# hasindu2008/cornetto

Hardware: AMD Instinct MI355X
Metric: Gbases/s scanned (telowin+sdust+boringbits) (higher is better)
Workload: dtype u8/u16 integer

## Files before the change

### cornetto_amd/__init__.py

```python
import ctypes as C
import os

import numpy as np

__all__ = ["lib", "Accel", "AccelError", "HIT_DT", "WIN_DT", "IVL_DT", "TELROW_DT", "khash_str_order", "panel_boring", "REG_DT", "REGREC_DT", "build",
           "LIB_PATH", "CLI_PATH"]

HERE = os.path.dirname(os.path.abspath(__file__))
DEV_LIB_PATH = os.path.join(HERE, "libcornetto_hip_dev.so")
LIB_PATH = os.environ.get("CORNETTO_LIB") or os.path.join(HERE, "libcornetto_hip.so")
CLI_PATH = os.path.join(HERE, "cornetto")

HIT_DT = np.dtype([("ctg", "<i4"), ("strand", "<i4"), ("start", "<i4"), ("end", "<i4")])
WIN_DT = np.dtype([("ctg", "<i4"), ("start", "<i4"), ("end", "<i4"), ("car", "<i4")])
IVL_DT = np.dtype([("ctg", "<i4"), ("start", "<i4"), ("finish", "<i4")])
TELROW_DT = np.dtype([("ctg", "<i4"), ("start", "<i4"), ("end", "<i4"), ("matched", "<i4")])
FQREC_DT = np.dtype([("head", "<i8"), ("seq", "<i8"), ("qual", "<i8"), ("len", "<i4"), ("name_len", "<i4"),
                     ("comment_len", "<i4"), ("keep", "<i4")])
EMITREC_DT = np.dtype([("ctg", "<i4"), ("rc", "<i4"), ("head", "<i8"), ("head_len", "<i8")])
FAREC_DT = np.dtype([("head", "<i8"), ("len", "<i8"), ("name_len", "<i4"), ("pad", "<i4")])
REG_DT = np.dtype([("st", "<i4"), ("end", "<i4"), ("depth", "<i4"), ("mq_depth", "<i4")])
REGREC_DT = np.dtype([("ctg", "<i4"), ("st", "<i4"), ("end", "<i4"), ("depth", "<i4"), ("mq_depth", "<i4")])
REGPK_DT = np.dtype([("st", "<i4"), ("depth", "<u2"), ("mq_depth", "<u2")])

# ... 343 lines not shown
    def telo_scan(self, asm, motif, thr_adj, want_hits=True):
        ph, nh, pw, nw = C.c_void_p(), C.c_int64(), C.c_void_p(), C.c_int64()
        self._chk(self.L.cornetto_telo_scan(self.h, asm.ptr, motif, thr_adj,
                                            C.byref(ph) if want_hits else None, C.byref(nh) if want_hits else None,
                                            C.byref(pw), C.byref(nw)))
        hits = _take(self.L, ph, nh.value, HIT_DT) if want_hits else None
        return hits, _take(self.L, pw, nw.value, WIN_DT)

    def sdust(self, asm, T=20, W=64):
        p, n = C.c_void_p(), C.c_int64()
        self._chk(self.L.cornetto_sdust_asm(self.h, asm.ptr, T, W, C.byref(p), C.byref(n)))
        return _take(self.L, p, n.value, IVL_DT)

    def sdust_begin(self, asm, T=20, W=64):
        self._chk(self.L.cornetto_sdust_asm_begin(self.h, asm.ptr, T, W))

    def sdust_end(self, asm, T=20, W=64):
        p, n = C.c_void_p(), C.c_int64()
        self._chk(self.L.cornetto_sdust_asm_end(self.h, asm.ptr, T, W, C.byref(p), C.byref(n)))
        return _take(self.L, p, n.value, IVL_DT)

    def sdust_stats(self, asm, T=20, W=64):
        self.L.cornetto_accel_sdust_stats(self.h, 1, None, 0)
        try:
            self.sdust(asm, T, W)
        finally:
            out = np.zeros(256, dtype=np.uint64)
            n = self.L.cornetto_accel_sdust_stats(self.h, 0, out.ctypes.data, 256)
        s = [int(x) for x in out[:n]]
        waves = s[254]
        if n > 207 and s[206]:
            return {"kernel": "sd_sift", "chunks": s[255], "tiles_of_64_bases": s[206], "positions_ct_above_T10": s[203], "after_L1": s[204], "after_L2": s[205],
                    "resolve_steps": s[200], "resolve_window_reads": s[201], "dp_tiles": s[208], "passes_with_candidates": s[202], "base_by_base_steps_of_chunks_with_other_bytes": s[207],
                    "window_reads_behind_a_gap_of": {"2": s[209], "3-4": s[210], "5-8": s[211]} if n > 211 else None}
        if not waves or not s[2]:
            return None
        hist = []
        for b in range(32):
            w = s[16 + 4 * b]
            if w:
                hist.append({"ms": [b * 0.5, b * 0.5 + 0.5], "waves": w, "jobs": s[18 + 4 * b], "find_perfect": s[19 + 4 * b], "find_perfect_with_candidates": s[17 + 4 * b]})
        return {"waves": waves, "chunks": s[255], "chunks_sampled_low_complexity": s[7], "wave_steps": s[2], "find_perfect_calls": s[3],
                "find_perfect_with_candidates": s[10], "plain_groups": s[4], "wave_ms_avg": round(s[5] / waves / 1e5, 3), "wave_ms_max": round(s[6] / 1e5, 3),
                "queue_fetch_rounds_per_wave": round(s[11] / waves, 1), "wave_time_histogram": hist}

    def cov_select_merged(self, cov, lo, hi, low_mq, edge_len, min_ctg_len, boring, merge_dist=1000, min_len=30000):
        p, n = C.c_void_p(), C.c_int64()
        self._chk(self.L.cornetto_cov_select_merged(self.h, cov.ptr, lo, hi, low_mq, edge_len, min_ctg_len, 1 if boring else 0, merge_dist, min_len,
                                                    C.byref(p), C.byref(n)))
        return _take(self.L, p, n.value, IVL_DT)

    def ivl_merge(self, ivls, dist):
        ivls = np.ascontiguousarray(ivls, dtype=IVL_DT)
        p, n = C.c_void_p(), C.c_int64()
        self._chk(self.L.cornetto_ivl_merge(self.h, ivls.ctypes.data, len(ivls), dist, C.byref(p), C.byref(n)))
        return _take(self.L, p, n.value, IVL_DT)

    def telobreaks(self, ctg_len, sd, tel):
        ctg_len = np.ascontiguousarray(ctg_len, dtype=np.int32)
        sd = np.ascontiguousarray(sd, dtype=IVL_DT)
        tel = np.ascontiguousarray(tel, dtype=TELROW_DT)
        p, n = C.c_void_p(), C.c_int64()
        self._chk(self.L.cornetto_telobreaks(self.h, ctg_len.ctypes.data, len(ctg_len), sd.ctypes.data, len(sd), tel.ctypes.data, len(tel),
                                             C.byref(p), C.byref(n)))
        return _take(self.L, p, n.value, IVL_DT)

    def cov_upload(self, depths, mqs):
# ... 164 lines not shown
```

### cornetto_amd/csrc/sdust.hip

```cpp
#include <algorithm>
#include <type_traits>
#include <ctime>
#include <sched.h>

#include "common.hpp"
#include "scan.hpp"
#include "tiles.hpp"
#include "ivlmerge.hpp"

namespace {

__device__ __forceinline__ int nt4_code(uint32_t c);
struct SdArgs;
struct SdChunk;
template <bool LEAN = false>
__device__ int sd_find_start(const SdArgs &A, const SdChunk ch, const uint8_t *seq);

struct SdChunk {
    int32_t ctg, start, end;
};
struct SdChunkFill {
    SdChunk *out;
    const int32_t *len;
    int32_t chunk;
// ... 1574 lines not shown
            uint32_t *d_slots = (uint32_t *)cn_ws(h, WS_SD_OFF, (size_t)(std::max<int64_t>(sd_waves, 1) + SD_WPB) * 64 * 64 * sizeof(uint32_t));
            if (!d_slots) return cn_fail(h, CORNETTO_E_NOMEM, "sdust: workspace allocation failed");
            stamp("row + slot workspaces");
            const bool use_w64 = w64_path;
            SdArgs A{a->d_bases, a->d_off, a->d_len, d_chunks, (int32_t)nc, T, W, d_out, d_cnt, (uint32_t)cap,
                     want_stats ? d_tot + 2 : nullptr, reinterpret_cast<uint32_t *>(d_tot + 1), d_slots, nullptr,
                     reinterpret_cast<uint32_t *>(d_tot + 8), nullptr, 0, CN_DEV_INT("CORNETTO_SDUST_RUNON", 1), (int32_t)chunk, a->d_wtab, a->d_wtab_base, reinterpret_cast<uint32_t *>(d_tot + 1) + 1};
            unsigned nb = (unsigned)((nc + 63) / 64);
            bool sift_walk_pending = false;
            bool dense_pending = false;
            struct DenseJoin {
                cornetto_accel_t *h;
                bool *pending;
                ~DenseJoin() { if (*pending && h->stream2) (void)hipStreamSynchronize(h->stream2); }
            } dense_join{h, &dense_pending};
            if (use_w64 && sift_on) {
                CN_HIP(h, hipMemsetAsync(d_cnt, 0, nc * 4, h->stream));
                const uint32_t reg_cap = (uint32_t)(chunk + 128);
                const uint32_t lds_wave = sift_lds_bytes(reg_cap);
                int lmin = 1;
                while (5 * (lmin + 1) <= T && lmin < 16) ++lmin;
                const bool walk_known = a->d_sd_walk && a->sd_walk_key == key;
                const size_t walk_words = 2 + 4 * nc + ((nc + 4095) / 4096 + 2);
                if (!walk_known) {
                    if (a->d_sd_walk) { (void)hipFree(a->d_sd_walk); a->d_sd_walk = nullptr; }
                    a->sd_walk_key = -1;
                    if (cn_obj_malloc(h, (void **)&a->d_sd_walk, walk_words * 4) != hipSuccess) return cn_fail(h, CORNETTO_E_NOMEM, "sdust: device allocation failed");
                    CN_HIP(h, hipMemsetAsync(a->d_sd_walk, 0, (2 + 2 * nc) * 4, h->stream));
                }
                uint32_t *d_wflag = a->d_sd_walk + 2 + nc, *d_wrank = d_wflag + nc, *d_worder = d_wrank + nc, *d_wpart = d_worder + nc;
                SiftArgs S{a->d_bases, a->d_off, a->d_len, d_chunks, (int32_t)nc, T, W, lds_wave, reg_cap,
                           walk_known ? d_worder : nullptr, walk_known ? nullptr : a->d_sd_walk, walk_known ? nullptr : d_wflag,
                           reinterpret_cast<uint32_t *>(d_tot + 256), T / 10 + 1, lmin, CN_DEV_INT("CORNETTO_SIFT_ABL", 0),
                           std::min(65, std::max(1, CN_DEV_INT("CORNETTO_SIFT_DP", 24))), std::min(65, std::max(1, CN_DEV_INT("CORNETTO_SIFT_L2SKIP", 48)))};
                sift_walk_pending = !walk_known;
                SdArgs R = A;
                R.stats = want_stats ? d_tot + 200 : nullptr;
                const bool cap_default = reg_cap == SIFT_CAP_DEFAULT && !CN_DEV_INT("CORNETTO_SIFT_GENERIC", 0) && !CN_DEV_INT("CORNETTO_SIFT_ABL", 0);
                if (h->sift_per_cu == 0 || h->sift_per_cu_default != (cap_default ? 1 : 0)) {
                    int per_cu = 0;
                    const hipError_t oe = cap_default ? hipOccupancyMaxActiveBlocksPerMultiprocessor(&per_cu, sd_sift<false, SIFT_CAP_DEFAULT>, 64 * SIFT_WPB, lds_wave * SIFT_WPB)
                                                      : hipOccupancyMaxActiveBlocksPerMultiprocessor(&per_cu, sd_sift<false>, 64 * SIFT_WPB, lds_wave * SIFT_WPB);
                    if (oe != hipSuccess || per_cu < 1) per_cu = 8;
                    h->sift_per_cu = per_cu;
                    h->sift_per_cu_default = cap_default ? 1 : 0;
                }
                const int per_cu_all = std::max(1, std::min<int>(h->sift_per_cu, (int)(163840 / ((lds_wave * SIFT_WPB + 1279) / 1280 * 1280))));
                const bool free_now = __atomic_load_n(&h->boost, __ATOMIC_ACQUIRE) != 0;
                const size_t cus_n = (size_t)std::max(h->sd_cus, 1);
                const size_t slots_all = (size_t)per_cu_all * cus_n;
                const size_t slots = free_now ? slots_all : std::max<size_t>(cus_n, slots_all * (size_t)h->share / 100);
                const size_t all_blocks = (nc + SIFT_WPB - 1) / SIFT_WPB;
                const unsigned nbk = (unsigned)std::min<size_t>(all_blocks, (size_t)CN_DEV_INT("CORNETTO_SIFT_BLOCKS", (int)slots));
                const unsigned extra = (unsigned)std::min<size_t>(all_blocks > nbk ? all_blocks - nbk : 0, slots_all > slots ? slots_all - slots : 0);
                const bool may_help = phase == 0 && extra > 0 && !want_stats && h->share < CN_DEV_INT("CORNETTO_SDUST_HELP_BELOW", 70);
                if (may_help) {
                    if (!h->stream2) {
                        int pr_least = 0, pr_greatest = 0;
                        (void)hipDeviceGetStreamPriorityRange(&pr_least, &pr_greatest);
                        CN_HIP(h, hipStreamCreateWithPriority(&h->stream2, hipStreamNonBlocking, pr_greatest));
                        CN_HIP(h, hipEventCreateWithFlags(&h->ev2, hipEventDisableTiming));
                        CN_HIP(h, hipEventCreateWithFlags(&h->ev1, hipEventDisableTiming));
                    }
                    if (!h->ev3) CN_HIP(h, hipEventCreateWithFlags(&h->ev3, hipEventDisableTiming));
                    CN_HIP(h, hipEventRecord(h->ev1, h->stream));
                }
                stamp("set up");
                if (want_stats) CN_LAUNCH(h, "sdust_kernel", sd_sift<true><<<dim3(nbk), dim3(64 * SIFT_WPB), lds_wave * SIFT_WPB, h->stream>>>(S, R));
                else if (cap_default) CN_LAUNCH(h, "sdust_kernel", sd_sift<false, SIFT_CAP_DEFAULT><<<dim3(nbk), dim3(64 * SIFT_WPB), lds_wave * SIFT_WPB, h->stream>>>(S, R));
                else CN_LAUNCH(h, "sdust_kernel", sd_sift<false><<<dim3(nbk), dim3(64 * SIFT_WPB), lds_wave * SIFT_WPB, h->stream>>>(S, R));
                __atomic_fetch_add(&h->launch_seq, 1ull, __ATOMIC_RELEASE);
                if (may_help) {
                    CN_HIP(h, hipEventRecord(h->ev3, h->stream));
                    bool helped = false;
                    while (hipEventQuery(h->ev3) == hipErrorNotReady) {
                        if (!helped && __atomic_load_n(&h->boost, __ATOMIC_ACQUIRE) != 0) {
                            CN_HIP(h, hipStreamWaitEvent(h->stream2, h->ev1, 0));
                            if (cap_default) sd_sift<false, SIFT_CAP_DEFAULT><<<dim3(extra), dim3(64 * SIFT_WPB), lds_wave * SIFT_WPB, h->stream2>>>(S, R);
                            else sd_sift<false><<<dim3(extra), dim3(64 * SIFT_WPB), lds_wave * SIFT_WPB, h->stream2>>>(S, R);
                            dense_pending = true;
                            CN_HIP(h, hipGetLastError());
                            CN_HIP(h, hipEventRecord(h->ev2, h->stream2));
                            helped = true;
                        }
                        sched_yield();
                    }
                    if (helped) CN_HIP(h, hipStreamWaitEvent(h->stream, h->ev2, 0));
// ... 138 lines not shown
                        cornetto_free(of);
                        return cn_fail(h, CORNETTO_E_HIP, "sdust: stitch / copy back failed");
                    }
                    if (phase == 1) {
                        h->sd_pend.state = 1; h->sd_pend.a = a; h->sd_pend.T = T; h->sd_pend.W = W; h->sd_pend.of = of;
                        h->sd_pend.m_cap = m_cap; h->sd_pend.n_cap = n_cap; h->sd_pend.cap = cap; h->sd_pend.key = key; h->sd_pend.walk_pending = sift_walk_pending;
                        return CORNETTO_OK;
                    }
                    const int fin = sd_one_go_finish(h, a, of, p_tot, cap, n_cap, m_cap, key, sift_walk_pending, ivls, n_ivls);
                    if (fin <= 0) {
                        if (fin == 0) stamp("results on the host (one go)");
                        return fin;
                    }
                } else if (of) {
                    cornetto_free(of);
                }
            }
            stamp("main kernel queued");
            CN_HIP(h, hipMemcpyAsync(p_tot, d_tot, want_stats ? 2048 : 128, hipMemcpyDeviceToHost, h->stream));
            CN_HIP(h, hipStreamSynchronize(h->stream));
            stamp("main kernel done");
            if (want_stats) {
                memcpy(h->sd_last, p_tot, 2048);
                if (a->sd_flagged >= 0) h->sd_last[7] = (unsigned long long)a->sd_flagged;
                h->sd_last[254] = nb;
                h->sd_last[255] = nc;
            }
            if (env_stats)
                for (int b = 0; b < 32; ++b)
                    if (p_tot[16 + 4 * b])
                        fprintf(stderr, "[sdust stats]   waves that ran %4.1f-%4.1f ms: %6llu, job fetches %llu, find_perfect calls %llu (%llu with candidates)\n", b * 0.5, b * 0.5 + 0.5,
                                p_tot[16 + 4 * b], p_tot[18 + 4 * b], p_tot[19 + 4 * b], p_tot[17 + 4 * b]);
            if (env_stats && sift_on)
                fprintf(stderr, "[sdust stats] sift: tiles %llu, positions with ct > T/10 %llu, after L1 %llu, after L2 %llu; resolve: steps %llu, window reads %llu (behind a gap of 2 / 3-4 / 5-8: %llu / %llu / %llu), dp tiles %llu; passes with candidates %llu; base-by-base steps of chunks with other bytes %llu\n",
                        p_tot[206], p_tot[203], p_tot[204], p_tot[205], p_tot[200], p_tot[201], p_tot[209], p_tot[210], p_tot[211], p_tot[208], p_tot[202], p_tot[207]);
            if (env_stats)
                fprintf(stderr, "[sdust stats] flagged low-complexity %llu; chunks %zu waves %u wave-steps %llu find_perfect calls %llu (%llu with candidates) plain groups %llu; wave time avg %.1f us max %.1f us; queue: %.1f fetch rounds and %.1f us per wave\n", p_tot[7], nc, nb,
                        p_tot[2], p_tot[3], p_tot[10], p_tot[4], nb ? (double)p_tot[5] / nb / 100.0 : 0.0, (double)p_tot[6] / 100.0, nb ? (double)p_tot[11] / nb : 0.0, nb ? (double)p_tot[12] / nb / 100.0 : 0.0);
            const uint32_t ovf = (uint32_t)(p_tot[1] & 0xFFFFFFFFull);
            const bool need_wtab = (p_tot[1] >> 32) != 0;
            if (need_wtab) {
                if (a->d_wtab) return cn_fail(h, CORNETTO_E_HIP, "sdust: word-count table requested twice");
                std::vector<int64_t> base(a->n + 1, 0);
                for (int32_t c = 0; c < a->n; ++c) base[c + 1] = base[c] + a->len[c] / SD_WBLK + 2;
                a->n_wblocks = base[a->n];
                const size_t npart = ((size_t)a->n_wblocks + 4095) / 4096 + 1;
                uint32_t *d_wcnt = nullptr;
                if (hipMalloc((void **)&a->d_wtab, ((size_t)a->n_wblocks + 1) * 4) != hipSuccess ||
                    hipMalloc((void **)&a->d_wtab_base, ((size_t)a->n + 1) * 8) != hipSuccess ||
                    hipMalloc((void **)&d_wcnt, ((size_t)a->n_wblocks + npart + 1) * 4) != hipSuccess)
                    return cn_fail(h, CORNETTO_E_NOMEM, "sdust: word-count table allocation failed");
                CN_HIP(h, hipMemcpyAsync(a->d_wtab_base, base.data(), ((size_t)a->n + 1) * 8, hipMemcpyHostToDevice, h->stream));
                const unsigned nbw = (unsigned)((a->n_wblocks + 255) / 256);
                CN_LAUNCH(h, "sd_wordcount", sd_wordcount<<<dim3(nbw), dim3(256), 0, h->stream>>>(a->d_bases, a->d_off, a->d_len, a->d_wtab_base, a->n,
                                                                                         a->n_wblocks, d_wcnt));
                int rc = cnscan::exclusive_u32(h, "sd_wordscan", d_wcnt, a->n_wblocks, 1, a->d_wtab, d_wcnt + a->n_wblocks, nullptr);
                hipError_t e = hipStreamSynchronize(h->stream);
                (void)hipFree(d_wcnt);
                if (rc != CORNETTO_OK) return rc;
                if (e != hipSuccess) return cn_fail(h, CORNETTO_E_HIP, "sdust: word-count table build failed");
                continue;
            }
            if (sift_walk_pending && !need_wtab) a->sd_walk_key = key;
            if (ovf <= cap) {
                tot = p_tot[0];
                break;
            }
            if (attempt >= 2) return cn_fail(h, CORNETTO_E_HIP, "sdust: a chunk produced %u intervals after resizing to %zu", ovf, cap);
// ... 168 lines not shown
```

### cornetto_amd/csrc/sdust_sift.hpp

```cpp
#pragma once

struct SiftArgs {
    const uint8_t *bases;
    const int64_t *ctg_off;
    const int32_t *ctg_len;
    const SdChunk *chunks;
    int32_t n_chunks;
    int32_t T, W;
    uint32_t lds_per_wave;
    uint32_t reg_cap;
    const uint32_t *order;
    uint32_t *walk_out;
    uint32_t *iswalk_out;
    uint32_t *counter;
    int32_t thr, lmin;
    int32_t abl;
    int32_t dp_min;
    int32_t l2_skip;
};

#ifndef SIFT_WPB
#define SIFT_WPB 1
#endif
constexpr int SIFT_NCTR = 64;
constexpr int SIFT_PAD = 16;
#ifndef SIFT_K
#define SIFT_K 16
#endif
constexpr int SIFT_LS = SIFT_K - 1;
constexpr int SIFT_FIXED = 1024 + 512;
__host__ __device__ constexpr uint32_t sift_lds_bytes(uint32_t cap) { return (SIFT_FIXED + cap / 4 + 2 * (SIFT_PAD + cap) + 16 + 15) / 16 * 16; }


__device__ __forceinline__ uint32_t sd_codes4(uint32_t word)
{
    const uint32_t y = word & 0xDFDFDFDFu, idx = y & 0x07070707u;
    const uint32_t code = __builtin_amdgcn_perm(0x02000003u, 0x01000000u, idx);
    const uint32_t d = y ^ __builtin_amdgcn_perm(0x47FFFF54u, 0x43FF41FFu, idx);
    const uint32_t nz = ((d & 0x7F7F7F7Fu) + 0x7F7F7F7Fu) | d;
    return code | ((nz >> 5) & 0x04040404u);
}
__device__ __forceinline__ uint32_t sd_words4(uint32_t cn, uint32_t pcn)
{
    const uint32_t y1 = __builtin_amdgcn_alignbyte(cn, pcn, 3);
    const uint32_t y2 = __builtin_amdgcn_alignbyte(cn, pcn, 2);
    const uint32_t t = (cn & 0x03030303u) | ((y1 & 0x03030303u) << 2) | ((y2 & 0x03030303u) << 4);
    return t | (((cn | y1 | y2) & 0x04040404u) << 4);
}

__device__ __forceinline__ int sd_mbcnt64(unsigned long long m)
{
    return (int)__builtin_amdgcn_mbcnt_hi((uint32_t)(m >> 32), __builtin_amdgcn_mbcnt_lo((uint32_t)m, 0u));
}
__device__ __forceinline__ int sd_dpp_shr1(int old, int src, bool zero_fill)
{
    return zero_fill ? __builtin_amdgcn_update_dpp(0, src, 0x138, 0xF, 0xF, true) : __builtin_amdgcn_update_dpp(old, src, 0x138, 0xF, 0xF, false);
}
// ... 56 lines not shown
    uint8_t *const wc = L + SIFT_FIXED + cap / 4 + 2 * SIFT_PAD;
    const int T = A.T, W = A.W, CAPW = W - 2;

    const int lo = lane - (CAPW - 1);
    const unsigned long long below = lane ? ~0ull >> (64 - lane) : 0ull;
    const unsigned long long mc = lo > 0 ? below & (~0ull << lo) : below;
    const unsigned long long mp = lo < 0 ? ~0ull << (64 + lo) : 0ull;
    const uint32_t m_a = (uint32_t)mc, m_d = (uint32_t)(mp >> 32), m_m = lane < 32 ? (uint32_t)mp : (uint32_t)(mc >> 32);
    const uint32_t mybit = 1u << (lane & 31);
    uint32_t *const mine0 = tab + (lane < 32 ? 0 : 192), *const mine1 = tab + (lane < 32 ? 64 : 128);
    uint32_t *const tab_mine = mine0;
    const uint32_t *const mid1 = tab + (lane < 32 ? 0 : 128);
    const int thr = A.thr, lmin = A.lmin;
    const int LS = CAPW - 1 < SIFT_LS ? CAPW - 1 : SIFT_LS;
    const bool long_ok = CAPW - 1 > LS;
    unsigned long long st_steps = 0, st_jumps = 0, st_cand = 0, st_trig = 0, st_l1 = 0, st_l2 = 0, st_walk = 0, st_tiles = 0, st_dp = 0, st_g2 = 0, st_g4 = 0, st_g8 = 0;

    struct Meta {
        SdChunk ch;
        int len;
        const uint8_t *seq;
    };
    struct Data {
        uint4 q[2];
        uint32_t pw[2];
    };
    auto meta = [&](int kk) {
        Meta m;
        m.ch = A.chunks[kk];
        m.len = A.ctg_len[m.ch.ctg];
        m.seq = A.bases + A.ctg_off[m.ch.ctg];
        return m;
    };
    auto fetch = [&](const Meta &m) {
        Data d;
        const int rb = m.ch.start - (m.ch.start > 0 ? 128 : 0), rlen = m.ch.end - rb;
#pragma unroll
        for (int it = 0; it < 2; ++it) {
            const int b16 = lane * 16 + it * 1024;
            d.q[it] = make_uint4(0, 0, 0, 0);
            if (b16 < rlen) d.q[it] = *reinterpret_cast<const uint4 *>(m.seq + rb + b16);
        }
        uint32_t first = 0;
        if (rb > 0) first = *reinterpret_cast<const uint32_t *>(m.seq + rb - 4);
        d.pw[0] = (uint32_t)__builtin_amdgcn_update_dpp((int)first, (int)d.q[0].w, 0x138, 0xF, 0xF, false);
        d.pw[1] = (uint32_t)__builtin_amdgcn_update_dpp(rdlane((int)d.q[0].w, 63), (int)d.q[1].w, 0x138, 0xF, 0xF, false);
        return d;
    };

  auto process = [&](const int k, const Meta &M, const Data &D) {
    const SdChunk ch = M.ch;
    const int len = M.len;
    const uint8_t *seq = M.seq;
    const int halo = ch.start > 0 ? 128 : 0;
    const int rb = ch.start - halo;
    const int rlen = ch.end - rb;
    const int ntile = (rlen + 63) >> 6;
    const bool islast = ch.end == len;
    const int rec_from = ch.start;

    tab[lane] = 0;
    tab[64 + lane] = 0;
    tab[128 + lane] = 0;
    tab[192 + lane] = 0;
    for (int i = lane; i < (int)(cap >> 4); i += 64) sb[i] = 0;
    if (lane < SIFT_PAD) reinterpret_cast<uint16_t *>(wc)[lane - SIFT_PAD] = halo ? 0xFF40 : 0x0040;
    bool bad = false;
    bool general = rb <= 0 || rb + ((rlen + 15) & ~15) > len || (abl & 32);
    if (abl & 128) general = false;
    if (!general && !(abl & 128)) {
        uint32_t acc = 0u;
        int lane_s = lane * 16;
        for (int b16 = lane * 16, it = 0; it < STAGE_ROUNDS && b16 < rlen; b16 += 1024, ++it) {
            uint4 q;
            uint32_t pw;
            if (STAGE_ROUNDS <= 2 || it < 2) {
                q = D.q[it];
                pw = D.pw[it];
            } else {
                asm volatile("" : "+v"(lane_s));
                const uint8_t *const g = seq + rb + lane_s + it * 1024;
                q = *reinterpret_cast<const uint4 *>(g);
                pw = *reinterpret_cast<const uint32_t *>(g - 4);
            }
            const uint32_t ipw = pw & 0x07070707u;
            uint32_t pcn = __builtin_amdgcn_perm(0x02000003u, 0x01000000u, ipw);
            acc |= (pw & 0xDFDFDFDFu) ^ __builtin_amdgcn_perm(0x47FFFF54u, 0x43FF41FFu, ipw);
            const uint32_t in[4] = {q.x, q.y, q.z, q.w};
            uint32_t wo[8];
#pragma unroll
            for (int d = 0; d < 4; ++d) {
                const uint32_t idx = in[d] & 0x07070707u;
                const uint32_t cn = __builtin_amdgcn_perm(0x02000003u, 0x01000000u, idx);
                acc |= (in[d] & 0xDFDFDFDFu) ^ __builtin_amdgcn_perm(0x47FFFF54u, 0x43FF41FFu, idx);
                const uint32_t y1 = __builtin_amdgcn_alignbyte(cn, pcn, 3), y2 = __builtin_amdgcn_alignbyte(cn, pcn, 2);
                const uint32_t w4 = cn | y1 << 2 | y2 << 4;
                wo[2 * d] = __builtin_amdgcn_perm(0u, w4, 0x0C010C00u);
                wo[2 * d + 1] = __builtin_amdgcn_perm(0u, w4, 0x0C030C02u);
                pcn = cn;
            }
            uint4 *dst = reinterpret_cast<uint4 *>(wc + 2 * b16);
            dst[0] = make_uint4(wo[0], wo[1], wo[2], wo[3]);
            dst[1] = make_uint4(wo[4], wo[5], wo[6], wo[7]);
        }
        general = sd_any(acc != 0u);
    }
    if (general)
    for (int b16 = lane * 16, it = 0; it < STAGE_ROUNDS && b16 < rlen; b16 += 1024, ++it) {
        const int p0 = rb + b16;
        uint4 q;
        uint32_t pw;
        if (STAGE_ROUNDS <= 2 || it < 2) {
            q = D.q[it];
            pw = D.pw[it];
        } else {
            q = *reinterpret_cast<const uint4 *>(seq + p0);
            pw = *reinterpret_cast<const uint32_t *>(seq + p0 - 4);
        }
        uint32_t pcn = 0x04040404u;
        if (p0 > 0) pcn = sd_codes4(pw);
        const uint32_t in[4] = {q.x, q.y, q.z, q.w};
        uint32_t wo[8];
#pragma unroll
        for (int d = 0; d < 4; ++d) {
            uint32_t cn = sd_codes4(in[d]);
            if (p0 + 4 * d + 4 > len) {
                const int rem = len - (p0 + 4 * d);
                const uint32_t beyond = rem <= 0 ? 0xFFFFFFFFu : 0xFFFFFFFFu << (8 * rem);
                bad = bad || (cn & 0x04040404u & ~beyond) != 0u;
                cn |= 0x04040404u & beyond;
            } else {
                bad = bad || (cn & 0x04040404u) != 0u;
            }
            const uint32_t w4 = sd_words4(cn, pcn);
            wo[2 * d] = __builtin_amdgcn_perm(0u, w4, 0x0C010C00u);
            wo[2 * d + 1] = __builtin_amdgcn_perm(0u, w4, 0x0C030C02u);
            pcn = cn;
        }
        uint4 *dst = reinterpret_cast<uint4 *>(wc + 2 * b16);
        dst[0] = make_uint4(wo[0], wo[1], wo[2], wo[3]);
        dst[1] = make_uint4(wo[4], wo[5], wo[6], wo[7]);
    }
    const bool unclean = sd_any(bad);
    SD_LDS_ORDER();

    int w = 0, r = 0, slot = 0;
    int sv0 = 0;
    bool have_last = false;
    uint32_t last_s = 0, last_f = 0, n_out = 0;
    uint2 *const out = O.out + (size_t)k * O.cap;
    auto emit = [&](int ps, int pf, int tm) {
        if (tm < rec_from) return;
        if (have_last && ps <= (int)last_f) {
            if (pf > (int)last_f) last_f = (uint32_t)pf;
        } else {
            if (have_last) {
                if (n_out < O.cap && lane == 0) out[n_out] = make_uint2(last_s, last_f);
                ++n_out;
            }
            have_last = true;
            last_s = (uint32_t)ps;
            last_f = (uint32_t)pf;
        }
    };
    auto emit_slots = [&](int from, int tm) {
        unsigned long long em = sd_ballot(slot != 0 && lane >= from && lane < CAPW);
        while (em) {
            const int a = 63 - __builtin_clzll(em);
            em &= ~(1ull << a);
            const uint32_t so = (uint32_t)rdlane(slot, a);
            const int s = sv0 - a;
            emit(s, s + (int)(so >> 24) + 3, tm);
        }
    };
    auto push_word = [&](int tw, int amax, bool age_slots) {
        const unsigned long long e = sd_ballot(w == tw) & ~(~1ull << (amax - 1 < 0 ? 0 : amax - 1)) & (amax > 0 ? ~0ull : 0ull);
        r = sd_dpp_shr1(0, r, true) + sd_mbcnt64(e);
        w = sd_dpp_shr1(tw, w, false);
        if (age_slots) slot = sd_dpp_shr1(0, slot, true);
    };
    auto pass = [&](int amax, const int Tl, const uint32_t m_recip) {
        const unsigned long long cm = sd_ballot(__mul24(r, 10) > Tl) & ~(~1ull << amax) & ~1ull;
        if (cm) {
            const bool cand = (cm >> lane) & 1ull;
            if (STATS) ++st_cand;
            uint32_t key_c = 0u;
            if (cand) key_c = lane == 1 ? ((uint32_t)r & 0x7FFu) << 13 : __umulhi(((uint32_t)r & 0x7FFu) << 13, m_recip);
            const uint32_t key_e = (uint32_t)slot & 0xFFFFFFu;
            const uint32_t xs = sd_scan_max_dpp(key_e > key_c ? key_e : key_c);
            const uint32_t sk = (uint32_t)__builtin_amdgcn_update_dpp(0, (int)xs, 0x138, 0xF, 0xF, true);
            const uint32_t km = sk > key_e ? sk : key_e;
            if (cand && key_c >= km) slot = (int)(key_c | ((uint32_t)lane << 24));
        }
    };
    auto finish = [&]() {
        if (have_last) {
            if (n_out < O.cap && lane == 0) out[n_out] = make_uint2(last_s, last_f);
            ++n_out;
        }
        if (lane == 0) {
            O.out_n[k] = n_out;
            if (n_out > O.cap) atomicMax(O.ovf, n_out);
            if (STATS) st_tiles += (unsigned long long)ntile;
        }
    };

    if (unclean) {
        const int Tl = T * lane;
        const uint32_t m_recip = sd_recip_tab[lane];
        if (A.walk_out && lane == 0) {
            A.iswalk_out[k] = 1u;
            A.walk_out[2 + atomicAdd(&A.walk_out[0], 1u)] = (uint32_t)k;
        }
        int u = sd_wave_find_start(ch, seq, W, lane);
        if (u == -2) u = __builtin_amdgcn_readfirstlane(sd_find_start<true>(O, ch, seq));
        if (u < 0) return;
        const int stop = islast ? len + 1 : ch.end;
        int l = 0, size = 0, cv = 4, ctile = -1;
        unsigned t = 0;
        for (int i = u; i < stop; ++i) {
            if ((i >> 6) != ctile) {
                ctile = i >> 6;
                const int p = ctile * 64 + lane;
                cv = p < len ? nt4_code(seq[p]) : 4;
            }
            const int b = rdlane(cv, i & 63);
            if (STATS) ++st_walk;
            if (b < 4) {
                ++l;
                t = (t << 2 | (unsigned)b) & 63u;
                if (l >= 3) {
                    const int start = (l - W > 0 ? l - W : 0) + (i + 1 - l);
                    const bool full = size >= CAPW;
                    const bool moves = l > W;
                    if (full && moves) {
                        const uint32_t so = (uint32_t)rdlane(slot, CAPW - 1);
// ... 115 lines not shown
            for (int j = 0; j < lmin; ++j) {
                d += 10 * (int)p[1 - 2 * j] - T;
                dmin = d < dmin ? d : dmin;
            }
        }
        const bool ok = on && dmin > 0;
        const unsigned long long m = sd_ballot(ok);
#ifdef SIFT_L2_ADAPT
        const bool hot = l2_hot >= 2 && __popcll(m) >= 16;
        if (hot && ++l2_skipped >= 12) l2_hot = 1;
        if (__popcll(m) >= A.l2_skip || hot) {
#else
        if (__popcll(m) >= A.l2_skip) {
#endif
            if (STATS) st_l1 += (unsigned long long)__popcll(m);
            if (STATS) st_l2 += (unsigned long long)__popcll(m);
            if (ok) (void)__hip_atomic_fetch_or(&sb[o >> 5], 1u << (o & 31), __ATOMIC_RELAXED, __HIP_MEMORY_SCOPE_WORKGROUP);
        } else if (m) {
            if (STATS) st_l1 += (unsigned long long)__popcll(m);
            if (ok) tl2[ntl2 + sd_mbcnt64(m)] = (uint16_t)o;
            ntl2 += __popcll(m);
            SD_LDS_ORDER();
            if (ntl2 >= 64) {
                run_l2(64);
                const uint16_t mv = tl2[64 + lane];
                SD_LDS_ORDER();
                tl2[lane] = mv;
                ntl2 -= 64;
                SD_LDS_ORDER();
            }
        }
    };

    uint8_t *pq = wc + 2 * lane;
    const uint32_t tab_a = (uint32_t)(uintptr_t)(lds_u32 *)tab, mine0_a = (uint32_t)(uintptr_t)(lds_u32 *)mine0, mine1_a = (uint32_t)(uintptr_t)(lds_u32 *)mine1,
                   mid1_a = (uint32_t)(uintptr_t)(lds_u32 *)mid1;
    auto lds_at = [](uint32_t wi, uint32_t base) __attribute__((always_inline)) {
        uint32_t a;
        asm("v_lshl_add_u32 %0, %1, 2, %2" : "=v"(a) : "v"(wi), "v"(base));
        return (lds_u32 *)(uintptr_t)a;
    };
    uint32_t wv_ahead = pq[0];
    auto tile = [&](auto par_c, auto general_c, auto only_c, const int q) __attribute__((always_inline)) {
        constexpr int PAR = decltype(par_c)::value;
        constexpr bool GENERAL = decltype(general_c)::value, TABLE_ONLY = decltype(only_c)::value;
        constexpr int A_AT = PAR ? 64 : 0, D_AT = PAR ? 192 : 128, M_AT = PAR ? 0 : 64;
        constexpr int Z0 = PAR ? 0 : 64, Z1 = PAR ? 192 : 128;
        constexpr bool CHECK = GENERAL || TABLE_ONLY;
        const uint32_t wv = wv_ahead;
        wv_ahead = pq[128];
        asm("" : "+v"(wv_ahead));
        const bool valid = !CHECK || (wv < 64u && q * 64 + lane < rlen);
        const uint32_t wi = CHECK ? wv & 63u : wv;
        lds_u32 *const t_mine = lds_at(wi, PAR ? mine1_a : mine0_a), *const t_all = lds_at(wi, tab_a), *const t_mid = lds_at(wi, mid1_a);
        if (valid) (void)__hip_atomic_fetch_or(t_mine, mybit, __ATOMIC_RELAXED, __HIP_MEMORY_SCOPE_WORKGROUP);
        SD_LDS_ORDER();
        const uint32_t e_a = t_all[A_AT], e_m = t_mid[M_AT], e_d = t_all[D_AT];
        SD_LDS_ORDER();
        tab[Z0 + lane] = 0;
        tab[Z1 + lane] = 0;
        uint32_t ctu = (uint32_t)__popc(e_a & m_a);
        asm("v_bcnt_u32_b32 %0, %1, %0" : "+v"(ctu) : "v"(e_m & m_m));
        asm("v_bcnt_u32_b32 %0, %1, %0" : "+v"(ctu) : "v"(e_d & m_d));
        const int ct = (int)ctu;
        pq[1] = (uint8_t)(TABLE_ONLY ? 255 : (valid ? ct : 0));
        pq += 128;
        if (!TABLE_ONLY) {
            const bool trig = valid && ct >= thr;
            const unsigned long long m = sd_ballot(trig);
            if (m) {
                if (STATS) st_trig += (unsigned long long)__popcll(m);
                int idx;
                asm("v_cndmask_b32_e64 %0, 64, %1, %2" : "=v"(idx) : "v"(sd_mbcnt64(m)), "s"(m));
                (tl + ntl)[idx] = (uint16_t)(q * 64 + lane);
                ntl += __popcll(m);
                SD_LDS_ORDER();
                if (ntl >= 64) {
                    if (!(abl & 2)) run_l1(64);
                    const uint16_t mv = tl[64 + lane];
                    SD_LDS_ORDER();
                    tl[lane] = mv;
                    ntl -= 64;
                    SD_LDS_ORDER();
                }
            }
        }
    };
    if (!(abl & 4)) {
        using P0 = std::integral_constant<int, 0>;
        using P1 = std::integral_constant<int, 1>;
        int q = 0;
        if (halo) tile(P0{}, std::false_type{}, std::true_type{}, q++);
        else tile(P0{}, std::true_type{}, std::false_type{}, q++);
        for (; q + 1 < ntile - 1; q += 2) {
            tile(P1{}, std::false_type{}, std::false_type{}, q);
            tile(P0{}, std::false_type{}, std::false_type{}, q + 1);
        }
        if (q < ntile - 1) { tile(P1{}, std::false_type{}, std::false_type{}, q); ++q; }
        if (q < ntile) {
            if (q & 1) tile(P1{}, std::true_type{}, std::false_type{}, q);
            else tile(P0{}, std::true_type{}, std::false_type{}, q);
        }
    }
    SD_LDS_ORDER();
    if (ntl > 0 && !(abl & 2)) run_l1(ntl);
    if (ntl2 > 0) run_l2(ntl2);
    if (abl & 1) { finish(); return; }
    SD_LDS_ORDER();

    const int s_lo = ch.start > 0 ? ch.start - W : -0x40000000, s_hi = islast ? 0x7fffffff : ch.end - W;
    int lane_r = lane;
    asm volatile("" : "+v"(lane_r));
    const int Tl = T * lane_r;
    const uint32_t m_recip = sd_recip_tab[lane_r];
    auto mark64 = [&](int o, int nbits) {
        const uint32_t d = (uint32_t)o >> 5, b = (uint32_t)o & 31u;
        const unsigned long long mk = nbits >= 64 ? ~0ull : (1ull << nbits) - 1ull;
        const unsigned long long lo64 = mk << b;
        const uint32_t w1 = (uint32_t)(lo64 >> 32), w2 = b ? (uint32_t)(mk >> (64u - b)) : 0u;
        (void)__hip_atomic_fetch_or(&cb[d], (uint32_t)lo64, __ATOMIC_RELAXED, __HIP_MEMORY_SCOPE_WORKGROUP);
        if (w1) (void)__hip_atomic_fetch_or(&cb[d + 1], w1, __ATOMIC_RELAXED, __HIP_MEMORY_SCOPE_WORKGROUP);
        if (w2) (void)__hip_atomic_fetch_or(&cb[d + 2], w2, __ATOMIC_RELAXED, __HIP_MEMORY_SCOPE_WORKGROUP);
    };
    auto mark = [&](int s, int nbits) {
        if (s < s_lo || s >= s_hi) return;
        if (nbits > 64) {
            mark64(s - rb, 64);
            mark64(s - rb + 64, nbits - 64);
        } else {
            mark64(s - rb, nbits);
        }
    };
    auto pass_m = [&](int amax) {
        const unsigned long long cm = sd_ballot(__mul24(r, 10) > Tl) & ~(~1ull << amax) & ~1ull;
// ... 190 lines not shown
        for (int base = 0; base <= nd; base += 64) {
            const int d = base + lane;
            const uint32_t v = d < nd ? cb[d] : 0u;
            const unsigned long long nz = sd_ballot(v != 0u);
            if (!nz && carry >= 0) {
                carry = 0;
                continue;
            }
            const uint32_t pm = (uint32_t)__builtin_amdgcn_update_dpp(carry, (int)v, 0x138, 0xF, 0xF, false) >> 31;
            const uint32_t sh = (v << 1) | pm;
            uint32_t st = v & ~sh, en = ~v & sh;
            const int ns = __popc(st), ne = __popc(en);
            const int xs = wave_scan_add(ns), xe = wave_scan_add(ne);
            uint32_t is = n_s + (uint32_t)(xs - ns), ie = n_e + (uint32_t)(xe - ne);
            while (st) {
                const int b = __builtin_ctz(st);
                st &= st - 1;
                if (is < O.cap) row[2 * is] = (uint32_t)(rb + 32 * d + b);
                ++is;
            }
            while (en) {
                const int b = __builtin_ctz(en);
                en &= en - 1;
                if (ie < O.cap) row[2 * ie + 1] = (uint32_t)(rb + 32 * d + b);
                ++ie;
            }
            n_s += (uint32_t)rdlane(xs, 63);
            n_e += (uint32_t)rdlane(xe, 63);
            carry = rdlane((int)v, 63);
        }
        if (lane == 0) {
            O.out_n[k] = n_s;
            if (n_s > O.cap) atomicMax(O.ovf, n_s);
            if (STATS) st_tiles += (unsigned long long)ntile;
        }
    }
  };

    int c = (int)((blockIdx.x * SIFT_WPB + wave) % SIFT_NCTR), dry = 0;
    auto ask = [&](int cc) {
        uint32_t v = 0;
        if (lane == 0) v = atomicAdd(&A.counter[cc * 16], 1u);
        return v;
    };
    uint32_t nxt = ask(c);
    for (;;) {
        const long long kk = (long long)__builtin_amdgcn_readfirstlane((int)nxt) * SIFT_NCTR + c;
        if (kk >= A.n_chunks) {
            static_assert(SIFT_NCTR == 64, "one lane per counter");
            if (dry < 2 * SIFT_NCTR) {
                const uint32_t seen = __hip_atomic_load(&A.counter[lane * 16], __ATOMIC_RELAXED, __HIP_MEMORY_SCOPE_AGENT);
                const long long left = (long long)A.n_chunks - lane;
                const unsigned long long open = sd_ballot(left > 0 && (long long)seen < (left + SIFT_NCTR - 1) / SIFT_NCTR);
                if (!open) break;
                ++dry;
                const int from = c + 1 == SIFT_NCTR ? 0 : c + 1;
                const unsigned long long rot = from ? (open >> from) | (open << (SIFT_NCTR - from)) : open;
                c = (from + __builtin_ctzll(rot)) & (SIFT_NCTR - 1);
                nxt = ask(c);
                continue;
            }
            if (++dry >= 3 * SIFT_NCTR) break;
            c = c + 1 == SIFT_NCTR ? 0 : c + 1;
            nxt = ask(c);
            continue;
        }
        dry = 0;
        nxt = ask(c);
        const int ko = A.order ? __builtin_amdgcn_readfirstlane((int)A.order[kk]) : (int)kk;
        const Meta m = meta(ko);
        process(ko, m, fetch(m));
    }
    if (STATS && O.stats && lane == 0) {
        atomicAdd(&O.stats[0], st_steps);
        atomicAdd(&O.stats[1], st_jumps);
        atomicAdd(&O.stats[2], st_cand);
        atomicAdd(&O.stats[3], st_trig);
        atomicAdd(&O.stats[4], st_l1);
        atomicAdd(&O.stats[5], st_l2);
        atomicAdd(&O.stats[6], st_tiles);
        atomicAdd(&O.stats[7], st_walk);
        atomicAdd(&O.stats[8], st_dp);
        atomicAdd(&O.stats[9], st_g2);
        atomicAdd(&O.stats[10], st_g4);
        atomicAdd(&O.stats[11], st_g8);
    }
}
```

Measured before the change: 490.5.

## Process runs of consecutive sift chunks per wave, reusing the seam halo

The sift work queue now hands out units that can be runs of several consecutive chunks, with a tail of single chunks kept for balance. When a chunk continues the previous one on the same contig, the wave skips re-fetching and re-staging the 128-base halo and carries the seam window counts and state bits over in LDS. It also skips the first halo tiles. This cuts redundant global loads and halo tile work but coarsens scheduling granularity, which risks worse load balance, and adds seam-handling complexity.

```diff
diff --git a/cornetto_amd/__init__.py b/cornetto_amd/__init__.py
--- a/cornetto_amd/__init__.py
+++ b/cornetto_amd/__init__.py
@@ -399,7 +399,8 @@
         if n > 207 and s[206]:
             return {"kernel": "sd_sift", "chunks": s[255], "tiles_of_64_bases": s[206], "positions_ct_above_T10": s[203], "after_L1": s[204], "after_L2": s[205],
                     "resolve_steps": s[200], "resolve_window_reads": s[201], "dp_tiles": s[208], "passes_with_candidates": s[202], "base_by_base_steps_of_chunks_with_other_bytes": s[207],
-                    "window_reads_behind_a_gap_of": {"2": s[209], "3-4": s[210], "5-8": s[211]} if n > 211 else None}
+                    "window_reads_behind_a_gap_of": {"2": s[209], "3-4": s[210], "5-8": s[211]} if n > 211 else None,
+                    "chunks_continued": s[212] if n > 212 else None}
         if not waves or not s[2]:
             return None
         hist = []
diff --git a/cornetto_amd/csrc/sdust.hip b/cornetto_amd/csrc/sdust.hip
--- a/cornetto_amd/csrc/sdust.hip
+++ b/cornetto_amd/csrc/sdust.hip
@@ -1630,7 +1630,8 @@
                 SiftArgs S{a->d_bases, a->d_off, a->d_len, d_chunks, (int32_t)nc, T, W, lds_wave, reg_cap,
                            walk_known ? d_worder : nullptr, walk_known ? nullptr : a->d_sd_walk, walk_known ? nullptr : d_wflag,
                            reinterpret_cast<uint32_t *>(d_tot + 256), T / 10 + 1, lmin, CN_DEV_INT("CORNETTO_SIFT_ABL", 0),
-                           std::min(65, std::max(1, CN_DEV_INT("CORNETTO_SIFT_DP", 24))), std::min(65, std::max(1, CN_DEV_INT("CORNETTO_SIFT_L2SKIP", 48)))};
+                           std::min(65, std::max(1, CN_DEV_INT("CORNETTO_SIFT_DP", 24))), std::min(65, std::max(1, CN_DEV_INT("CORNETTO_SIFT_L2SKIP", 48))),
+                           std::min(64, std::max(1, CN_DEV_INT("CORNETTO_SIFT_RUN", SIFT_RUN))), 0, walk_known ? a->d_sd_walk : nullptr};
                 sift_walk_pending = !walk_known;
                 SdArgs R = A;
                 R.stats = want_stats ? d_tot + 200 : nullptr;
@@ -1651,6 +1652,7 @@
                 const size_t all_blocks = (nc + SIFT_WPB - 1) / SIFT_WPB;
                 const unsigned nbk = (unsigned)std::min<size_t>(all_blocks, (size_t)CN_DEV_INT("CORNETTO_SIFT_BLOCKS", (int)slots));
                 const unsigned extra = (unsigned)std::min<size_t>(all_blocks > nbk ? all_blocks - nbk : 0, slots_all > slots ? slots_all - slots : 0);
+                S.tail = (int32_t)std::min<size_t>(nc, (size_t)nbk * SIFT_WPB * (size_t)S.run);
                 const bool may_help = phase == 0 && extra > 0 && !want_stats && h->share < CN_DEV_INT("CORNETTO_SDUST_HELP_BELOW", 70);
                 if (may_help) {
                     if (!h->stream2) {
@@ -1855,8 +1857,8 @@
                         fprintf(stderr, "[sdust stats]   waves that ran %4.1f-%4.1f ms: %6llu, job fetches %llu, find_perfect calls %llu (%llu with candidates)\n", b * 0.5, b * 0.5 + 0.5,
                                 p_tot[16 + 4 * b], p_tot[18 + 4 * b], p_tot[19 + 4 * b], p_tot[17 + 4 * b]);
             if (env_stats && sift_on)
-                fprintf(stderr, "[sdust stats] sift: tiles %llu, positions with ct > T/10 %llu, after L1 %llu, after L2 %llu; resolve: steps %llu, window reads %llu (behind a gap of 2 / 3-4 / 5-8: %llu / %llu / %llu), dp tiles %llu; passes with candidates %llu; base-by-base steps of chunks with other bytes %llu\n",
-                        p_tot[206], p_tot[203], p_tot[204], p_tot[205], p_tot[200], p_tot[201], p_tot[209], p_tot[210], p_tot[211], p_tot[208], p_tot[202], p_tot[207]);
+                fprintf(stderr, "[sdust stats] sift: tiles %llu, positions with ct > T/10 %llu, after L1 %llu, after L2 %llu; resolve: steps %llu, window reads %llu (behind a gap of 2 / 3-4 / 5-8: %llu / %llu / %llu), dp tiles %llu; passes with candidates %llu; base-by-base steps of chunks with other bytes %llu; chunks that continued the one before %llu\n",
+                        p_tot[206], p_tot[203], p_tot[204], p_tot[205], p_tot[200], p_tot[201], p_tot[209], p_tot[210], p_tot[211], p_tot[208], p_tot[202], p_tot[207], p_tot[212]);
             if (env_stats)
                 fprintf(stderr, "[sdust stats] flagged low-complexity %llu; chunks %zu waves %u wave-steps %llu find_perfect calls %llu (%llu with candidates) plain groups %llu; wave time avg %.1f us max %.1f us; queue: %.1f fetch rounds and %.1f us per wave\n", p_tot[7], nc, nb,
                         p_tot[2], p_tot[3], p_tot[10], p_tot[4], nb ? (double)p_tot[5] / nb / 100.0 : 0.0, (double)p_tot[6] / 100.0, nb ? (double)p_tot[11] / nb : 0.0, nb ? (double)p_tot[12] / nb / 100.0 : 0.0);
diff --git a/cornetto_amd/csrc/sdust_sift.hpp b/cornetto_amd/csrc/sdust_sift.hpp
--- a/cornetto_amd/csrc/sdust_sift.hpp
+++ b/cornetto_amd/csrc/sdust_sift.hpp
@@ -17,12 +17,17 @@
     int32_t abl;
     int32_t dp_min;
     int32_t l2_skip;
+    int32_t run, tail;
+    const uint32_t *n_first;
 };
 
 #ifndef SIFT_WPB
 #define SIFT_WPB 1
 #endif
 constexpr int SIFT_NCTR = 64;
+#ifndef SIFT_RUN
+#define SIFT_RUN 4
+#endif
 constexpr int SIFT_PAD = 16;
 #ifndef SIFT_K
 #define SIFT_K 16
@@ -145,9 +150,11 @@
         m.seq = A.bases + A.ctg_off[m.ch.ctg];
         return m;
     };
-    auto fetch = [&](const Meta &m) {
+    int pv_ctg = -1, pv_end = 0, pv_rlen = 0;
+    unsigned long long st_cont = 0;
+    auto fetch = [&](const Meta &m, const bool cont) {
         Data d;
-        const int rb = m.ch.start - (m.ch.start > 0 ? 128 : 0), rlen = m.ch.end - rb;
+        const int rb = m.ch.start - (m.ch.start > 0 && !cont ? 128 : 0), rlen = m.ch.end - rb;
 #pragma unroll
         for (int it = 0; it < 2; ++it) {
             const int b16 = lane * 16 + it * 1024;
@@ -161,7 +168,7 @@
         return d;
     };
 
-  auto process = [&](const int k, const Meta &M, const Data &D) {
+  auto process = [&](const int k, const Meta &M, const Data &D, const bool cont) {
     const SdChunk ch = M.ch;
     const int len = M.len;
     const uint8_t *seq = M.seq;
@@ -171,12 +178,30 @@
     const int ntile = (rlen + 63) >> 6;
     const bool islast = ch.end == len;
     const int rec_from = ch.start;
-
+    const int soff = cont ? 128 : 0;
+    const int slen = rlen - soff;
+    const int from_rlen = pv_rlen;
+    pv_ctg = -1;
+
+    uint32_t seam_wc = 0, seam_sb = 0;
+    int lane_c = lane;
+    if (cont) {
+        asm volatile("" : "+v"(lane_c));
+        seam_wc = reinterpret_cast<const uint32_t *>(wc)[((from_rlen - 128) >> 1) + lane_c];
+        if (lane_c < 2) seam_sb = sb[2 * ((from_rlen >> 6) - 1) + lane_c];
+        SD_LDS_ORDER();
+    }
     tab[lane] = 0;
     tab[64 + lane] = 0;
     tab[128 + lane] = 0;
     tab[192 + lane] = 0;
     for (int i = lane; i < (int)(cap >> 4); i += 64) sb[i] = 0;
+    if (cont) {
+        SD_LDS_ORDER();
+        reinterpret_cast<uint32_t *>(wc)[lane_c] = seam_wc;
+        if (lane_c < 2) sb[2 + lane_c] = seam_sb;
+        if (STATS) ++st_cont;
+    }
     if (lane < SIFT_PAD) reinterpret_cast<uint16_t *>(wc)[lane - SIFT_PAD] = halo ? 0xFF40 : 0x0040;
     bool bad = false;
     bool general = rb <= 0 || rb + ((rlen + 15) & ~15) > len || (abl & 32);
@@ -184,7 +209,7 @@
     if (!general && !(abl & 128)) {
         uint32_t acc = 0u;
         int lane_s = lane * 16;
-        for (int b16 = lane * 16, it = 0; it < STAGE_ROUNDS && b16 < rlen; b16 += 1024, ++it) {
+        for (int b16 = lane * 16, it = 0; it < STAGE_ROUNDS && b16 < slen; b16 += 1024, ++it) {
             uint4 q;
             uint32_t pw;
             if (STAGE_ROUNDS <= 2 || it < 2) {
@@ -192,7 +217,7 @@
                 pw = D.pw[it];
             } else {
                 asm volatile("" : "+v"(lane_s));
-                const uint8_t *const g = seq + rb + lane_s + it * 1024;
+                const uint8_t *const g = seq + rb + soff + lane_s + it * 1024;
                 q = *reinterpret_cast<const uint4 *>(g);
                 pw = *reinterpret_cast<const uint32_t *>(g - 4);
             }
@@ -212,15 +237,15 @@
                 wo[2 * d + 1] = __builtin_amdgcn_perm(0u, w4, 0x0C030C02u);
                 pcn = cn;
             }
-            uint4 *dst = reinterpret_cast<uint4 *>(wc + 2 * b16);
+            uint4 *dst = reinterpret_cast<uint4 *>(wc + 2 * (b16 + soff));
             dst[0] = make_uint4(wo[0], wo[1], wo[2], wo[3]);
             dst[1] = make_uint4(wo[4], wo[5], wo[6], wo[7]);
         }
         general = sd_any(acc != 0u);
     }
     if (general)
-    for (int b16 = lane * 16, it = 0; it < STAGE_ROUNDS && b16 < rlen; b16 += 1024, ++it) {
-        const int p0 = rb + b16;
+    for (int b16 = lane * 16, it = 0; it < STAGE_ROUNDS && b16 < slen; b16 += 1024, ++it) {
+        const int p0 = rb + soff + b16;
         uint4 q;
         uint32_t pw;
         if (STAGE_ROUNDS <= 2 || it < 2) {
@@ -250,7 +275,7 @@
             wo[2 * d + 1] = __builtin_amdgcn_perm(0u, w4, 0x0C030C02u);
             pcn = cn;
         }
-        uint4 *dst = reinterpret_cast<uint4 *>(wc + 2 * b16);
+        uint4 *dst = reinterpret_cast<uint4 *>(wc + 2 * (b16 + soff));
         dst[0] = make_uint4(wo[0], wo[1], wo[2], wo[3]);
         dst[1] = make_uint4(wo[4], wo[5], wo[6], wo[7]);
     }
@@ -314,7 +339,7 @@
         if (lane == 0) {
             O.out_n[k] = n_out;
             if (n_out > O.cap) atomicMax(O.ovf, n_out);
-            if (STATS) st_tiles += (unsigned long long)ntile;
+            if (STATS) st_tiles += (unsigned long long)(ntile - (soff >> 6));
         }
     };
 
@@ -496,7 +521,7 @@
         }
     };
 
-    uint8_t *pq = wc + 2 * lane;
+    uint8_t *pq = wc + 2 * lane + 2 * soff;
     const uint32_t tab_a = (uint32_t)(uintptr_t)(lds_u32 *)tab, mine0_a = (uint32_t)(uintptr_t)(lds_u32 *)mine0, mine1_a = (uint32_t)(uintptr_t)(lds_u32 *)mine1,
                    mid1_a = (uint32_t)(uintptr_t)(lds_u32 *)mid1;
     auto lds_at = [](uint32_t wi, uint32_t base) __attribute__((always_inline)) {
@@ -554,16 +579,25 @@
         using P0 = std::integral_constant<int, 0>;
         using P1 = std::integral_constant<int, 1>;
         int q = 0;
-        if (halo) tile(P0{}, std::false_type{}, std::true_type{}, q++);
+        if (cont) {
+            int lane_t = lane;
+            asm volatile("" : "+v"(lane_t));
+            const uint32_t w1 = wc[2 * (64 + lane_t)];
+            if (w1 < 64u) (void)__hip_atomic_fetch_or(lds_at(w1, mine0_a), mybit, __ATOMIC_RELAXED, __HIP_MEMORY_SCOPE_WORKGROUP);
+            q = 2;
+        }
+        else if (halo) tile(P0{}, std::false_type{}, std::true_type{}, q++);
         else tile(P0{}, std::true_type{}, std::false_type{}, q++);
         for (; q + 1 < ntile - 1; q += 2) {
             tile(P1{}, std::false_type{}, std::false_type{}, q);
             tile(P0{}, std::false_type{}, std::false_type{}, q + 1);
         }
-        if (q < ntile - 1) { tile(P1{}, std::false_type{}, std::false_type{}, q); ++q; }
-        if (q < ntile) {
-            if (q & 1) tile(P1{}, std::true_type{}, std::false_type{}, q);
-            else tile(P0{}, std::true_type{}, std::false_type{}, q);
+        if (q < ntile - 1) {
+            tile(P1{}, std::false_type{}, std::false_type{}, q);
+            ++q;
+            if (q < ntile) tile(P0{}, std::true_type{}, std::false_type{}, q);
+        } else if (q < ntile) {
+            tile(P1{}, std::true_type{}, std::false_type{}, q);
         }
     }
     SD_LDS_ORDER();
@@ -820,11 +854,30 @@
         if (lane == 0) {
             O.out_n[k] = n_s;
             if (n_s > O.cap) atomicMax(O.ovf, n_s);
-            if (STATS) st_tiles += (unsigned long long)ntile;
-        }
+            if (STATS) st_tiles += (unsigned long long)(ntile - (soff >> 6));
+        }
+    }
+    if (!(rlen & 63) && rlen >= 128 && !abl) {
+        pv_ctg = ch.ctg;
+        pv_end = ch.end;
+        pv_rlen = rlen;
     }
   };
 
+#ifdef CN_DEV
+    const int RUN = A.run;
+#else
+    constexpr int RUN = SIFT_RUN;
+#endif
+    auto unit_plan = [&](int &n_first, int &n_runs) {
+        n_first = 0;
+        if (A.order) {
+            n_first = (int)__builtin_amdgcn_readfirstlane((int)A.n_first[0]);
+            n_first = n_first < A.n_chunks ? n_first : A.n_chunks;
+        }
+        const int mid = A.n_chunks - n_first - A.tail;
+        n_runs = mid > 0 ? mid / RUN : 0;
+    };
     int c = (int)((blockIdx.x * SIFT_WPB + wave) % SIFT_NCTR), dry = 0;
     auto ask = [&](int cc) {
         uint32_t v = 0;
@@ -832,13 +885,18 @@
         return v;
     };
     uint32_t nxt = ask(c);
+    int kk = 0, todo = 0;
     for (;;) {
-        const long long kk = (long long)__builtin_amdgcn_readfirstlane((int)nxt) * SIFT_NCTR + c;
-        if (kk >= A.n_chunks) {
+      if (todo == 0) {
+        const long long u = (long long)__builtin_amdgcn_readfirstlane((int)nxt) * SIFT_NCTR + c;
+        int n_first, n_runs;
+        unit_plan(n_first, n_runs);
+        const int n_units = A.n_chunks - n_runs * (RUN - 1);
+        if (u >= n_units) {
             static_assert(SIFT_NCTR == 64, "one lane per counter");
             if (dry < 2 * SIFT_NCTR) {
                 const uint32_t seen = __hip_atomic_load(&A.counter[lane * 16], __ATOMIC_RELAXED, __HIP_MEMORY_SCOPE_AGENT);
-                const long long left = (long long)A.n_chunks - lane;
+                const long long left = (long long)n_units - lane;
                 const unsigned long long open = sd_ballot(left > 0 && (long long)seen < (left + SIFT_NCTR - 1) / SIFT_NCTR);
                 if (!open) break;
                 ++dry;
@@ -855,9 +913,22 @@
         }
         dry = 0;
         nxt = ask(c);
-        const int ko = A.order ? __builtin_amdgcn_readfirstlane((int)A.order[kk]) : (int)kk;
+        const int ui = (int)u;
+        const bool isrun = ui >= n_first && ui < n_first + n_runs;
+        kk = ui < n_first ? ui : isrun ? n_first + (ui - n_first) * RUN : ui + n_runs * (RUN - 1);
+        todo = isrun ? RUN : 1;
+        pv_ctg = -1;
+      }
+        const int ko = A.order ? __builtin_amdgcn_readfirstlane((int)A.order[kk]) : kk;
         const Meta m = meta(ko);
-        process(ko, m, fetch(m));
+#ifdef BIS_A
+        const bool cont = false;
+#else
+        const bool cont = pv_ctg == m.ch.ctg && pv_end == m.ch.start;
+#endif
+        ++kk;
+        --todo;
+        process(ko, m, fetch(m, cont), cont);
     }
     if (STATS && O.stats && lane == 0) {
         atomicAdd(&O.stats[0], st_steps);
@@ -872,5 +943,6 @@
         atomicAdd(&O.stats[9], st_g2);
         atomicAdd(&O.stats[10], st_g4);
         atomicAdd(&O.stats[11], st_g8);
+        atomicAdd(&O.stats[12], st_cont);
     }
 }
```

Result: faster. 497.6 (median of 4 runs) (+1.4%).
